# llm-d-incubation/workload-variant-autoscaler

Measured on AMD Instinct MI355X. Metric: solver_wall_clock_ms, lower is better.
Workload: dtype fp64; 1 GPU; model=3 models x 2 service classes (config #3), variants=64, accelerator_types=3, global_batch=64, seq_len=0, parallelism=fleet-shard dp1, analyzer_device=cuda

## Files before the change

### wva_amd/csrc/queue_solver.cpp

```cpp

#include <torch/extension.h>

#ifdef WVA_WITH_HIP
#include <c10/hip/HIPStream.h>
#endif

#include <climits>
#include <cmath>
#include <vector>


#include "queue_host.h"

#ifdef WVA_WITH_HIP
extern "C" int wva_launch_solve(const double *prob, double *out, int n_problems,
                                int max_k, void *stream);
#endif

static torch::Tensor solve_allocations(torch::Tensor problems, int64_t max_k_hint = -1) {
  TORCH_CHECK(problems.dim() == 2 && problems.size(1) == wva::PROBLEM_FIELDS,
              "problems must be [B, ", (int)wva::PROBLEM_FIELDS, "]");
  TORCH_CHECK(problems.scalar_type() == torch::kFloat64, "problems must be float64");
  problems = problems.contiguous();
  const int64_t B = problems.size(0);
  auto out = torch::zeros({B, (int64_t)wva::RESULT_FIELDS}, problems.options());
  if (B == 0) return out;

  if (problems.is_cuda()) {
#ifdef WVA_WITH_HIP
    int max_k;
    if (max_k_hint > 0) {
      max_k = max_k_hint > INT_MAX ? INT_MAX : (int)max_k_hint;
    } else {
      auto n = problems.select(1, wva::P_MAX_BATCH);
      auto in_range = n.ge(1.0).logical_and(n.lt((double)wva::kMaxBatchLimit + 1.0));
      const double max_batch =
          torch::where(in_range, n, torch::ones_like(n)).max().item<double>();
      max_k = (int)max_batch * (1 + wva::kMaxQueueToBatchRatio);
    }
    auto stream = c10::hip::getCurrentHIPStream();
    const int status = wva_launch_solve(problems.data_ptr<double>(),
                                        out.data_ptr<double>(), (int)B, max_k,
                                        (void *)stream.stream());
    TORCH_CHECK(status != -1,
                "max_batch too large for the LDS-resident GPU path (limit ~700, "
                "chain length ", max_k, "); use the CPU path for these problems");
    TORCH_CHECK(status == 0, "wva sizing kernel launch failed: ",
                hipGetErrorString((hipError_t)status));
    return out;
#else
    TORCH_CHECK(false, "wva native extension built without HIP support");
#endif
  }

  const double *pr = problems.data_ptr<double>();
  double *res = out.data_ptr<double>();
  int max_k = 1;
  for (int64_t i = 0; i < B; ++i) {
    int k = wva::row_chain_length(pr + i * wva::PROBLEM_FIELDS);
    if (k > max_k) max_k = k;
  }
  at::parallel_for(0, B, 1, [&](int64_t begin, int64_t end) {
    std::vector<double> cum((size_t)max_k);
    for (int64_t i = begin; i < end; ++i) {
      wva::solve_one(pr + i * wva::PROBLEM_FIELDS, res + i * wva::RESULT_FIELDS,
                     cum.data());
    }
  });
  return out;
}

PYBIND11_MODULE(TORCH_EXTENSION_NAME, m) {
  m.doc() = "wva_amd native batched queue solver (CPU + gfx950 HIP)";
  m.def("solve_allocations", &solve_allocations,
        "Batched state-dependent M/M/1/K allocation sizing",
        pybind11::arg("problems"), pybind11::arg("max_k_hint") = -1);
  m.attr("PROBLEM_FIELDS") = (int)wva::PROBLEM_FIELDS;
  m.attr("RESULT_FIELDS") = (int)wva::RESULT_FIELDS;
#ifdef WVA_WITH_HIP
  m.attr("HAS_HIP") = true;
#else
  m.attr("HAS_HIP") = false;
#endif
}
```

### wva_amd/ops/batched.py

```python

from __future__ import annotations

import math
from typing import Dict, List, Optional, Tuple

import numpy as np

from ..analyzer import (
    AnalyzerError,
    Configuration,
    DecodeParms,
    PrefillParms,
    QueueAnalyzer,
    RequestSize,
    ServiceParms,
    TargetPerf,
)
from ..config import MAX_QUEUE_TO_BATCH_RATIO
from ..core import Allocation, System
from ..core.allocation import _zero_load_allocation, energy_value_term

P_ALPHA, P_BETA, P_GAMMA, P_DELTA = 0, 1, 2, 3
P_IN_TOKENS, P_OUT_TOKENS, P_MAX_BATCH = 4, 5, 6
P_TARGET_TTFT, P_TARGET_ITL, P_TARGET_TPS = 7, 8, 9
P_TOTAL_RATE, P_MIN_REPLICAS = 10, 11
PROBLEM_FIELDS = 12

R_FEASIBLE, R_REPLICAS, R_RATE_STAR, R_ITL, R_TTFT, R_RHO = range(6)
RESULT_FIELDS = 6

GPU_MAX_BATCH_LIMIT = 700

_MAX_BATCH_LIMIT = (2**31 - 1) // (1 + MAX_QUEUE_TO_BATCH_RATIO)


def valid_rows(problems: np.ndarray) -> np.ndarray:
    p = problems
    with np.errstate(invalid="ignore"):
        ok = np.isfinite(p).all(axis=1)
        ok &= (p[:, P_ALPHA : P_DELTA + 1] >= 0).all(axis=1)
        ok &= (p[:, P_MAX_BATCH] >= 1) & (p[:, P_MAX_BATCH] < _MAX_BATCH_LIMIT + 1)
        ok &= (p[:, P_OUT_TOKENS] >= 1) & (p[:, P_OUT_TOKENS] < 2.0**31)
        ok &= p[:, P_IN_TOKENS] >= 0
        ok &= (p[:, P_TARGET_TTFT : P_TARGET_TPS + 1] >= 0).all(axis=1)
    return ok

_graph_cache: dict = {}
_graph_lock = None
_graph_disabled = False
_mg1_warned = False


def _graph_solve(native, problems_t, max_k):
    global _graph_lock, _graph_disabled
    import os
    import threading

    if _graph_disabled or os.environ.get("WVA_GPU_GRAPH", "0") != "1":
        return None
    import torch

    if _graph_lock is None:
        _graph_lock = threading.Lock()
    key = (problems_t.shape[0], max_k)
    with _graph_lock:
        entry = _graph_cache.get(key)
        try:
            if entry is None:
                if len(_graph_cache) >= 16:
                    _graph_cache.pop(next(iter(_graph_cache)))
                static_in = problems_t.clone()
                side = torch.cuda.Stream()
                side.wait_stream(torch.cuda.current_stream())
                with torch.cuda.stream(side):
                    native.solve_allocations(static_in, max_k)
                torch.cuda.current_stream().wait_stream(side)
                graph = torch.cuda.CUDAGraph()
                with torch.cuda.graph(graph):
                    static_out = native.solve_allocations(static_in, max_k)
                _graph_cache[key] = (graph, static_in, static_out)
                graph.replay()
                return static_out.cpu().numpy()
            graph, static_in, static_out = entry
            static_in.copy_(problems_t)
            graph.replay()
            return static_out.cpu().numpy()
        except Exception as e:
            _graph_disabled = True
            import logging

            logging.getLogger("wva").warning(
                "hipGraph dispatch unavailable; using plain launches: %s", e
            )
            return None


def _solve_problems_python(problems: np.ndarray, scv=1.0) -> np.ndarray:
    scv_arr = np.broadcast_to(np.asarray(scv, dtype=np.float64), (problems.shape[0],))
    out = np.zeros((problems.shape[0], RESULT_FIELDS), dtype=np.float64)
    valid = valid_rows(problems)
    for i, row in enumerate(problems):
        if not valid[i]:
            continue
        N = int(row[P_MAX_BATCH])
        config = Configuration(
            max_batch_size=N,
            max_queue_size=N * MAX_QUEUE_TO_BATCH_RATIO,
            service_parms=ServiceParms(
                prefill=PrefillParms(gamma=row[P_GAMMA], delta=row[P_DELTA]),
                decode=DecodeParms(alpha=row[P_ALPHA], beta=row[P_BETA]),
            ),
        )
        try:
            qa = QueueAnalyzer(
                config,
                RequestSize(
                    avg_input_tokens=int(row[P_IN_TOKENS]),
                    avg_output_tokens=int(row[P_OUT_TOKENS]),
                ),
                scv=float(scv_arr[i]),
            )
            _, metrics, _ = qa.size(
                TargetPerf(
                    target_ttft=row[P_TARGET_TTFT],
                    target_itl=row[P_TARGET_ITL],
                    target_tps=row[P_TARGET_TPS],
                )
            )
            rate_star = metrics.throughput
            total_rate = row[P_TOTAL_RATE]
            n_rep = max(math.ceil(total_rate / rate_star), int(row[P_MIN_REPLICAS]))
            if n_rep <= 0:
                continue
            final = qa.analyze(total_rate / n_rep)
        except AnalyzerError:
            continue
        out[i, R_FEASIBLE] = 1.0
        out[i, R_REPLICAS] = n_rep
        out[i, R_RATE_STAR] = rate_star
        out[i, R_ITL] = final.avg_token_time
        out[i, R_TTFT] = final.avg_wait_time + final.avg_prefill_time
        out[i, R_RHO] = final.rho
    return out


def solve_problems(problems: np.ndarray, device: Optional[str] = None) -> np.ndarray:
    from . import get_native, native_available

    problems = np.ascontiguousarray(problems, dtype=np.float64)
    if problems.ndim != 2 or problems.shape[1] != PROBLEM_FIELDS:
        raise ValueError(f"problems must be [B, {PROBLEM_FIELDS}]")
    if problems.shape[0] == 0:
        return np.zeros((0, RESULT_FIELDS), dtype=np.float64)

    from ..analyzer.mg1 import configured_scv

    scv = configured_scv()
    if scv != 1.0:
        global _mg1_warned
        if not _mg1_warned:
            _mg1_warned = True
            import logging

            logging.getLogger("wva_amd.ops").info(
                "WVA_ANALYZER=mg1 (cs^2=%.3g): sizing via the Python "
                "M/G/1-corrected analyzer instead of the native kernel", scv,
            )
        return _solve_problems_python(problems, scv=scv)

    want_gpu = device is not None and str(device).startswith("cuda")
    if want_gpu:
        native = get_native()
        import torch

        batch_limits = problems[:, P_MAX_BATCH]
        max_batch = batch_limits.max()
        if not max_batch <= GPU_MAX_BATCH_LIMIT:
            batch_limits = np.where(valid_rows(problems), batch_limits, 1.0)
            max_batch = batch_limits.max()
        if max_batch > GPU_MAX_BATCH_LIMIT:
            big = batch_limits > GPU_MAX_BATCH_LIMIT
            out = np.empty((problems.shape[0], RESULT_FIELDS), dtype=np.float64)
            out[~big] = solve_problems(problems[~big], device=device)
            out[big] = solve_problems(problems[big], device="cpu")
            return out
        max_k = max(int(max_batch), 1) * (1 + MAX_QUEUE_TO_BATCH_RATIO)
        t = torch.from_numpy(problems).to(device)
        res = _graph_solve(native, t, max_k)
        if res is not None:
            return res
        return native.solve_allocations(t, max_k).cpu().numpy()

    from . import get_native_cpu, native_cpu_available

    if native_cpu_available():
        return get_native_cpu().solve_allocations(problems)
    if native_available():
        import torch

        native = get_native()
        return native.solve_allocations(torch.from_numpy(problems)).numpy()
    from . import warn_if_pure_python_fallback

    warn_if_pure_python_fallback()
    return _solve_problems_python(problems)


class BatchedAllocationSolver:

    def __init__(self, device: Optional[str] = None) -> None:
        self.device = device

    def calculate(self, system: System) -> None:
        for g in system.accelerators.values():
            g.calculate()

        pair_cache: Dict[Tuple[str, str], Optional[Tuple[float, float, float, float, int, int, float]]] = {}

        def pair_info(model, acc):
            key = (model.name, acc.name)
            hit = pair_cache.get(key, False)
            if hit is not False:
                return hit
            perf = model.get_perf_data(acc.name)
            if perf is None:
                pair_cache[key] = None
                return None
            info = (
                perf.decode_parms.alpha,
                perf.decode_parms.beta,
                perf.prefill_parms.gamma,
                perf.prefill_parms.delta,
                perf.max_batch_size,
                perf.at_tokens,
                acc.cost * model.get_num_instances(acc.name),
            )
            pair_cache[key] = info
            return info

        from ..core.allocation import sizing_headroom

        headroom_factor = 1.0 + sizing_headroom()
        rows: List[Tuple[float, ...]] = []
        keys: List[Tuple[str, str, int]] = []
        zero_load: Dict[str, Dict[str, Allocation]] = {}
        costs: List[float] = []
        scv_rows: List[float] = []
        rows_append, keys_append, costs_append = rows.append, keys.append, costs.append
        scv_append = scv_rows.append

        for server in system.servers.values():
            server.all_allocations = {}
            load = server.load
            if (
                load is None
                or load.arrival_rate < 0
                or load.avg_in_tokens < 0
                or load.avg_out_tokens < 0
            ):
                continue
            model = system.model(server.model_name)
            if model is None:
                continue
            svc = system.service_class(server.service_class_name)
            if svc is None:
                continue
            target = svc.model_target(server.model_name)
            if target is None:
                continue
            target_ttft, target_itl, target_tps = target.ttft, target.itl, target.tps
            arrival, in_tok, out_tok = load.arrival_rate, load.avg_in_tokens, load.avg_out_tokens
            server_name = server.name
            server_max_batch = server.max_batch_size
            min_replicas = float(server.min_num_replicas)
            candidates = server.get_candidate_accelerators(system.accelerators)
            for acc in candidates.values():
                info = pair_info(model, acc)
                if info is None:
                    continue
                if arrival == 0 or out_tok == 0:
                    perf = model.get_perf_data(acc.name)
                    alloc = _zero_load_allocation(server, model, acc, perf)
                    zero_load.setdefault(server_name, {})[acc.name] = alloc
                    continue
                alpha, beta, gamma, delta, perf_max_batch, at_tokens, cost_per_rep = info
                K = int(out_tok)
                N = server_max_batch if server_max_batch > 0 else max(perf_max_batch * at_tokens // K, 1)
                total_rate = (
                    arrival / 60.0 if target_tps == 0 else target_tps / float(K)
                ) * headroom_factor
                rows_append(
                    (alpha, beta, gamma, delta, float(int(in_tok)), float(K), float(N),
                     target_ttft, target_itl, target_tps, total_rate, min_replicas)
                )
                keys_append((server_name, acc.name, N))
                costs_append(cost_per_rep)
                scv_append(getattr(server, "service_scv", -1.0))

        if rows:
            arr = np.array(rows, dtype=np.float64)
            from ..analyzer.mg1 import configured_scv

            global_scv = configured_scv()
            scv_arr = np.array(
                [s if s >= 0 else global_scv for s in scv_rows], dtype=np.float64
            )
            if (scv_arr != 1.0).any():
                results = _solve_problems_python(arr, scv=scv_arr)
            else:
                results = solve_problems(arr, self.device)
        else:
            results = np.zeros((0, RESULT_FIELDS))

        opt_spec = system.optimizer_spec
        energy_enabled = (
            opt_spec is not None
            and opt_spec.objective == "cost+energy"
            and opt_spec.energy_cost_per_kwh > 0
        )
        servers = system.servers
        results_list = results.tolist()
        for (server_name, acc_name, N), res, cost_per_replica in zip(keys, results_list, costs):
            if res[R_FEASIBLE] != 1.0:
                continue
            server = servers[server_name]
            num_replicas = int(res[R_REPLICAS])
            alloc = Allocation(
                accelerator=acc_name,
                num_replicas=num_replicas,
                batch_size=N,
                cost=cost_per_replica * num_replicas,
                itl=res[R_ITL],
                ttft=res[R_TTFT],
                rho=res[R_RHO],
                max_arrv_rate_per_replica=res[R_RATE_STAR] / 1000.0,
            )
            cur = server.cur_allocation
            alloc.value = cur.transition_penalty(alloc) if cur is not None else alloc.cost
            if energy_enabled:
                alloc.value += energy_value_term(system, server, alloc)
            server.all_allocations[acc_name] = alloc

        for server_name, accs in zero_load.items():
            server = servers[server_name]
            for acc_name, alloc in accs.items():
                if server.cur_allocation is not None:
                    alloc.set_value(server.cur_allocation.transition_penalty(alloc))
                if energy_enabled:
                    alloc.set_value(alloc.value + energy_value_term(system, server, alloc))
                server.all_allocations[acc_name] = alloc
```

Before: 931.4 us.

## Add pinned-buffer async GPU dispatch and chunk host row building over kernel

Adds a native submit/collect path that keeps a pool of pinned host and device buffers on a private non-blocking stream, so upload, the sizing kernel and download are queued without torch tensor allocation or a device sync per call. The batched solver splits servers into chunks (two by default for small fleets) so Python row building and result application for one chunk overlap with the GPU solve of the other. The CUDA output tensor also switches from zeros to empty. The cost is more complexity, per-slot lifetime state, and an extra kernel launch per chunk, which can outweigh the overlap when the fleet is small.

```diff
diff --git a/wva_amd/csrc/queue_solver.cpp b/wva_amd/csrc/queue_solver.cpp
--- a/wva_amd/csrc/queue_solver.cpp
+++ b/wva_amd/csrc/queue_solver.cpp
@@ -15,6 +15,8 @@
 #ifdef WVA_WITH_HIP
 extern "C" int wva_launch_solve(const double *prob, double *out, int n_problems,
                                 int max_k, void *stream);
+
+#include "sizing_dispatch.h"
 #endif
 
 static torch::Tensor solve_allocations(torch::Tensor problems, int64_t max_k_hint = -1) {
@@ -23,7 +25,9 @@
   TORCH_CHECK(problems.scalar_type() == torch::kFloat64, "problems must be float64");
   problems = problems.contiguous();
   const int64_t B = problems.size(0);
-  auto out = torch::zeros({B, (int64_t)wva::RESULT_FIELDS}, problems.options());
+  auto out = problems.is_cuda()
+                 ? torch::empty({B, (int64_t)wva::RESULT_FIELDS}, problems.options())
+                 : torch::zeros({B, (int64_t)wva::RESULT_FIELDS}, problems.options());
   if (B == 0) return out;
 
   if (problems.is_cuda()) {
@@ -78,6 +82,16 @@
   m.attr("PROBLEM_FIELDS") = (int)wva::PROBLEM_FIELDS;
   m.attr("RESULT_FIELDS") = (int)wva::RESULT_FIELDS;
 #ifdef WVA_WITH_HIP
+  m.def("submit", &wva::dispatch::submit,
+        "Enqueue upload, sizing kernel and download for a float64 [B, 12] "
+        "numpy array on the private dispatch stream; returns a ticket "
+        "without waiting",
+        pybind11::arg("problems"), pybind11::arg("max_k"));
+  m.def("collect", &wva::dispatch::collect,
+        "Wait (GIL released) for a ticket and return its float64 [B, 6] results",
+        pybind11::arg("ticket"));
+  m.def("dispatch_pool_stats", &wva::dispatch::pool_stats,
+        "(slots, slots in flight) of the dispatch pool");
   m.attr("HAS_HIP") = true;
 #else
   m.attr("HAS_HIP") = false;
diff --git a/wva_amd/csrc/sizing_dispatch.h b/wva_amd/csrc/sizing_dispatch.h
--- /dev/null
+++ b/wva_amd/csrc/sizing_dispatch.h
@@ -0,0 +1,228 @@
+
+#pragma once
+
+#include <hip/hip_runtime.h>
+#include <pybind11/numpy.h>
+#include <pybind11/pybind11.h>
+
+#include <climits>
+#include <cstdint>
+#include <cstring>
+#include <mutex>
+#include <stdexcept>
+#include <string>
+#include <unordered_set>
+#include <vector>
+
+#include "queue_core.h"
+
+extern "C" int wva_launch_solve(const double *prob, double *out, int n_problems,
+                                int max_k, void *stream);
+
+namespace wva {
+namespace dispatch {
+
+namespace py = pybind11;
+
+inline void hip_check(hipError_t err, const char *what) {
+  if (err != hipSuccess) {
+    throw std::runtime_error(std::string("wva sizing dispatch: ") + what +
+                             " failed: " + hipGetErrorString(err));
+  }
+}
+
+struct DeviceGuard {
+  int prev = -1;
+  bool switched = false;
+  explicit DeviceGuard(int device) {
+    hip_check(hipGetDevice(&prev), "hipGetDevice");
+    if (prev != device) {
+      hip_check(hipSetDevice(device), "hipSetDevice");
+      switched = true;
+    }
+  }
+  ~DeviceGuard() {
+    if (switched) (void)hipSetDevice(prev);
+  }
+};
+
+enum class SlotState { kFree, kInFlight, kCollecting };
+
+struct Slot {
+  double *h_in = nullptr;
+  double *h_out = nullptr;
+  double *d_in = nullptr;
+  double *d_out = nullptr;
+  int64_t cap_rows = 0;
+  hipEvent_t done = nullptr;
+  SlotState state = SlotState::kFree;
+  int64_t ticket = 0;
+  int64_t rows = 0;
+};
+
+struct Pool {
+  std::mutex mu;
+  int device = -1;
+  hipStream_t stream = nullptr;
+  std::vector<Slot *> slots;
+  std::unordered_set<int64_t> empty_tickets;
+  int64_t next_ticket = 1;
+};
+
+inline Pool &pool() {
+  static Pool *p = new Pool();
+  return *p;
+}
+
+inline void grow_slot(Slot &s, int64_t rows) {
+  if (rows <= s.cap_rows) return;
+  if (s.h_in) (void)hipHostFree(s.h_in);
+  if (s.h_out) (void)hipHostFree(s.h_out);
+  if (s.d_in) (void)hipFree(s.d_in);
+  if (s.d_out) (void)hipFree(s.d_out);
+  s.h_in = s.h_out = s.d_in = s.d_out = nullptr;
+  s.cap_rows = 0;
+  const int64_t cap = (rows + 255) / 256 * 256;
+  const size_t in_bytes = (size_t)cap * PROBLEM_FIELDS * sizeof(double);
+  const size_t out_bytes = (size_t)cap * RESULT_FIELDS * sizeof(double);
+  hip_check(hipHostMalloc((void **)&s.h_in, in_bytes, hipHostMallocDefault),
+            "hipHostMalloc");
+  hip_check(hipHostMalloc((void **)&s.h_out, out_bytes, hipHostMallocDefault),
+            "hipHostMalloc");
+  hip_check(hipMalloc((void **)&s.d_in, in_bytes), "hipMalloc");
+  hip_check(hipMalloc((void **)&s.d_out, out_bytes), "hipMalloc");
+  s.cap_rows = cap;
+}
+
+inline int64_t submit(py::array problems, int64_t max_k) {
+  if (!py::isinstance<py::array_t<double>>(problems)) {
+    throw py::type_error("problems must be a float64 array");
+  }
+  if (problems.ndim() != 2 || problems.shape(1) != PROBLEM_FIELDS) {
+    throw py::value_error("problems must be [B, " +
+                          std::to_string((int)PROBLEM_FIELDS) + "]");
+  }
+  if (!(problems.flags() & py::array::c_style)) {
+    throw py::value_error("problems must be C-contiguous");
+  }
+  const int64_t B = problems.shape(0);
+  if (B > INT_MAX) throw py::value_error("too many problems for one launch");
+
+  Pool &P = pool();
+  std::lock_guard<std::mutex> lock(P.mu);
+  if (B == 0) {
+    const int64_t ticket = P.next_ticket++;
+    P.empty_tickets.insert(ticket);
+    return ticket;
+  }
+  if (P.device < 0) hip_check(hipGetDevice(&P.device), "hipGetDevice");
+  DeviceGuard guard(P.device);
+  if (P.stream == nullptr) {
+    hip_check(hipStreamCreateWithFlags(&P.stream, hipStreamNonBlocking),
+              "hipStreamCreateWithFlags");
+  }
+
+  Slot *slot = nullptr;
+  for (Slot *s : P.slots) {
+    if (s->state == SlotState::kFree) {
+      slot = s;
+      break;
+    }
+  }
+  if (slot == nullptr) {
+    Slot *s = new Slot();
+    hipError_t err = hipEventCreateWithFlags(&s->done, hipEventDisableTiming);
+    if (err != hipSuccess) {
+      delete s;
+      hip_check(err, "hipEventCreateWithFlags");
+    }
+    P.slots.push_back(s);
+    slot = s;
+  }
+  grow_slot(*slot, B);
+
+  const size_t in_bytes = (size_t)B * PROBLEM_FIELDS * sizeof(double);
+  const size_t out_bytes = (size_t)B * RESULT_FIELDS * sizeof(double);
+  std::memcpy(slot->h_in, problems.data(), in_bytes);
+  hip_check(hipMemcpyAsync(slot->d_in, slot->h_in, in_bytes,
+                           hipMemcpyHostToDevice, P.stream),
+            "hipMemcpyAsync (upload)");
+  const int k = max_k > INT_MAX ? INT_MAX : (max_k < 0 ? 0 : (int)max_k);
+  const int status =
+      wva_launch_solve(slot->d_in, slot->d_out, (int)B, k, (void *)P.stream);
+  if (status != 0) {
+    (void)hipStreamSynchronize(P.stream);
+    if (status == -1) {
+      throw std::runtime_error(
+          "no kernel geometry holds a chain of length " + std::to_string(max_k) +
+          " in LDS (max_batch limit ~700); use the CPU path for these problems");
+    }
+    hip_check((hipError_t)status, "sizing kernel launch");
+  }
+  hipError_t err = hipMemcpyAsync(slot->h_out, slot->d_out, out_bytes,
+                                  hipMemcpyDeviceToHost, P.stream);
+  if (err == hipSuccess) err = hipEventRecord(slot->done, P.stream);
+  if (err != hipSuccess) {
+    (void)hipStreamSynchronize(P.stream);
+    hip_check(err, "hipMemcpyAsync (download) / hipEventRecord");
+  }
+  slot->state = SlotState::kInFlight;
+  slot->ticket = P.next_ticket++;
+  slot->rows = B;
+  return slot->ticket;
+}
+
+inline std::vector<py::ssize_t> result_shape(int64_t rows) {
+  return {(py::ssize_t)rows, (py::ssize_t)RESULT_FIELDS};
+}
+
+inline py::array_t<double> collect(int64_t ticket) {
+  Pool &P = pool();
+  Slot *slot = nullptr;
+  {
+    std::lock_guard<std::mutex> lock(P.mu);
+    if (P.empty_tickets.erase(ticket)) {
+      return py::array_t<double>(result_shape(0));
+    }
+    for (Slot *s : P.slots) {
+      if (s->ticket == ticket && s->state != SlotState::kFree) {
+        slot = s;
+        break;
+      }
+    }
+    if (slot == nullptr || slot->state == SlotState::kCollecting) {
+      const bool issued = ticket >= 1 && ticket < P.next_ticket;
+      throw py::value_error(
+          (issued ? "sizing ticket already collected: " : "unknown sizing ticket: ") +
+          std::to_string(ticket));
+    }
+    slot->state = SlotState::kCollecting;
+  }
+  const int64_t rows = slot->rows;
+  py::array_t<double> out(result_shape(rows));
+  double *dst = out.mutable_data();
+  hipError_t err;
+  {
+    py::gil_scoped_release nogil;
+    err = hipEventSynchronize(slot->done);
+    if (err == hipSuccess) {
+      std::memcpy(dst, slot->h_out, (size_t)rows * RESULT_FIELDS * sizeof(double));
+    }
+    std::lock_guard<std::mutex> lock(P.mu);
+    slot->state = SlotState::kFree;
+    slot->ticket = 0;
+  }
+  hip_check(err, "hipEventSynchronize");
+  return out;
+}
+
+inline py::tuple pool_stats() {
+  Pool &P = pool();
+  std::lock_guard<std::mutex> lock(P.mu);
+  int64_t busy = 0;
+  for (Slot *s : P.slots) busy += s->state != SlotState::kFree;
+  return py::make_tuple((int64_t)P.slots.size(), busy);
+}
+
+}
+}
diff --git a/wva_amd/ops/batched.py b/wva_amd/ops/batched.py
--- a/wva_amd/ops/batched.py
+++ b/wva_amd/ops/batched.py
@@ -1,7 +1,9 @@
 
 from __future__ import annotations
 
+import contextlib
 import math
+import os
 from typing import Dict, List, Optional, Tuple
 
 import numpy as np
@@ -51,9 +53,23 @@
 _mg1_warned = False
 
 
+def _graph_requested() -> bool:
+    return not _graph_disabled and os.environ.get("WVA_GPU_GRAPH", "0") == "1"
+
+
+_NO_DEVICE_SWITCH = contextlib.nullcontext()
+
+
+def _on_device(device):
+    if str(device) == "cuda":
+        return _NO_DEVICE_SWITCH
+    import torch
+
+    return torch.cuda.device(torch.device(device))
+
+
 def _graph_solve(native, problems_t, max_k):
     global _graph_lock, _graph_disabled
-    import os
     import threading
 
     if _graph_disabled or os.environ.get("WVA_GPU_GRAPH", "0") != "1":
@@ -185,11 +201,13 @@
             out[big] = solve_problems(problems[big], device="cpu")
             return out
         max_k = max(int(max_batch), 1) * (1 + MAX_QUEUE_TO_BATCH_RATIO)
-        t = torch.from_numpy(problems).to(device)
-        res = _graph_solve(native, t, max_k)
-        if res is not None:
-            return res
-        return native.solve_allocations(t, max_k).cpu().numpy()
+        if _graph_requested():
+            t = torch.from_numpy(problems).to(device)
+            res = _graph_solve(native, t, max_k)
+            if res is not None:
+                return res
+        with _on_device(device):
+            return native.collect(native.submit(problems, max_k))
 
     from . import get_native_cpu, native_cpu_available
 
@@ -206,14 +224,87 @@
     return _solve_problems_python(problems)
 
 
+class SyncDispatch:
+
+    def __init__(self, device: Optional[str], global_scv: Optional[float] = None) -> None:
+        self.device = device
+        self.global_scv = global_scv
+
+    def submit(self, problems: np.ndarray, scv_rows=None):
+        if self.global_scv is not None:
+            scv_arr = np.array(
+                [s if s >= 0 else self.global_scv for s in scv_rows], dtype=np.float64
+            )
+            if (scv_arr != 1.0).any():
+                return _solve_problems_python(problems, scv=scv_arr)
+        return solve_problems(problems, self.device)
+
+    def collect(self, ticket) -> np.ndarray:
+        return ticket
+
+
+class NativeGpuDispatch:
+
+    def __init__(self, native, device: str) -> None:
+        self.native = native
+        self.device = device
+
+    def submit(self, problems: np.ndarray, scv_rows=None):
+        max_batch = problems[:, P_MAX_BATCH].max()
+        if not max_batch <= GPU_MAX_BATCH_LIMIT:
+            return None, solve_problems(problems, self.device)
+        max_k = max(int(max_batch), 1) * (1 + MAX_QUEUE_TO_BATCH_RATIO)
+        with _on_device(self.device):
+            return self.native.submit(problems, max_k), None
+
+    def collect(self, ticket) -> np.ndarray:
+        native_ticket, solved = ticket
+        if native_ticket is None:
+            return solved
+        return self.native.collect(native_ticket)
+
+
+DEFAULT_GPU_CHUNKS = 2
+
+_GPU_CHUNKING_ROW_BOUND = 512
+
+
 class BatchedAllocationSolver:
 
-    def __init__(self, device: Optional[str] = None) -> None:
+    def __init__(self, device: Optional[str] = None, chunks: Optional[int] = None) -> None:
+        if chunks is not None and chunks < 1:
+            raise ValueError("chunks must be at least 1")
         self.device = device
+        self.chunks = chunks
+
+    def _plan(self, system: System, servers):
+        from ..analyzer.mg1 import configured_scv
+
+        global_scv = configured_scv()
+        if global_scv != 1.0 or any(
+            s >= 0 and s != 1.0 for s in [getattr(v, "service_scv", -1.0) for v in servers]
+        ):
+            return SyncDispatch(self.device, global_scv), 1, True
+        want_gpu = self.device is not None and str(self.device).startswith("cuda")
+        if want_gpu and not _graph_requested():
+            from . import get_native
+
+            native = get_native()
+            if native is None or not native.HAS_HIP:
+                raise RuntimeError("the native HIP extension is required for device "
+                                   f"{self.device!r} and is not built")
+            chunks = self.chunks if self.chunks is not None else DEFAULT_GPU_CHUNKS
+            if len(servers) * len(system.accelerators) >= _GPU_CHUNKING_ROW_BOUND:
+                chunks = 1
+            return NativeGpuDispatch(native, self.device), chunks, False
+        return SyncDispatch(self.device), self.chunks or 1, False
 
     def calculate(self, system: System) -> None:
         for g in system.accelerators.values():
             g.calculate()
+
+        all_servers = list(system.servers.values())
+        dispatch, n_chunks, track_scv = self._plan(system, all_servers)
 
         pair_cache: Dict[Tuple[str, str], Optional[Tuple[float, float, float, float, int, int, float]]] = {}
 
@@ -241,77 +332,7 @@
         from ..core.allocation import sizing_headroom
 
         headroom_factor = 1.0 + sizing_headroom()
-        rows: List[Tuple[float, ...]] = []
-        keys: List[Tuple[str, str, int]] = []
-        zero_load: Dict[str, Dict[str, Allocation]] = {}
-        costs: List[float] = []
-        scv_rows: List[float] = []
-        rows_append, keys_append, costs_append = rows.append, keys.append, costs.append
-        scv_append = scv_rows.append
-
-        for server in system.servers.values():
-            server.all_allocations = {}
-            load = server.load
-            if (
-                load is None
-                or load.arrival_rate < 0
-                or load.avg_in_tokens < 0
-                or load.avg_out_tokens < 0
-            ):
-                continue
-            model = system.model(server.model_name)
-            if model is None:
-                continue
-            svc = system.service_class(server.service_class_name)
-            if svc is None:
-                continue
-            target = svc.model_target(server.model_name)
-            if target is None:
-                continue
-            target_ttft, target_itl, target_tps = target.ttft, target.itl, target.tps
-            arrival, in_tok, out_tok = load.arrival_rate, load.avg_in_tokens, load.avg_out_tokens
-            server_name = server.name
-            server_max_batch = server.max_batch_size
-            min_replicas = float(server.min_num_replicas)
-            candidates = server.get_candidate_accelerators(system.accelerators)
-            for acc in candidates.values():
-                info = pair_info(model, acc)
-                if info is None:
-                    continue
-                if arrival == 0 or out_tok == 0:
-                    perf = model.get_perf_data(acc.name)
-                    alloc = _zero_load_allocation(server, model, acc, perf)
-                    zero_load.setdefault(server_name, {})[acc.name] = alloc
-                    continue
-                alpha, beta, gamma, delta, perf_max_batch, at_tokens, cost_per_rep = info
-                K = int(out_tok)
-                N = server_max_batch if server_max_batch > 0 else max(perf_max_batch * at_tokens // K, 1)
-                total_rate = (
-                    arrival / 60.0 if target_tps == 0 else target_tps / float(K)
-                ) * headroom_factor
-                rows_append(
-                    (alpha, beta, gamma, delta, float(int(in_tok)), float(K), float(N),
-                     target_ttft, target_itl, target_tps, total_rate, min_replicas)
-                )
-                keys_append((server_name, acc.name, N))
-                costs_append(cost_per_rep)
-                scv_append(getattr(server, "service_scv", -1.0))
-
-        if rows:
-            arr = np.array(rows, dtype=np.float64)
-            from ..analyzer.mg1 import configured_scv
-
-            global_scv = configured_scv()
-            scv_arr = np.array(
-                [s if s >= 0 else global_scv for s in scv_rows], dtype=np.float64
-            )
-            if (scv_arr != 1.0).any():
-                results = _solve_problems_python(arr, scv=scv_arr)
-            else:
-                results = solve_problems(arr, self.device)
-        else:
-            results = np.zeros((0, RESULT_FIELDS))
-
+        accelerators = system.accelerators
         opt_spec = system.optimizer_spec
         energy_enabled = (
             opt_spec is not None
@@ -319,33 +340,124 @@
             and opt_spec.energy_cost_per_kwh > 0
         )
         servers = system.servers
-        results_list = results.tolist()
-        for (server_name, acc_name, N), res, cost_per_replica in zip(keys, results_list, costs):
-            if res[R_FEASIBLE] != 1.0:
-                continue
-            server = servers[server_name]
-            num_replicas = int(res[R_REPLICAS])
-            alloc = Allocation(
-                accelerator=acc_name,
-                num_replicas=num_replicas,
-                batch_size=N,
-                cost=cost_per_replica * num_replicas,
-                itl=res[R_ITL],
-                ttft=res[R_TTFT],
-                rho=res[R_RHO],
-                max_arrv_rate_per_replica=res[R_RATE_STAR] / 1000.0,
-            )
-            cur = server.cur_allocation
-            alloc.value = cur.transition_penalty(alloc) if cur is not None else alloc.cost
-            if energy_enabled:
-                alloc.value += energy_value_term(system, server, alloc)
-            server.all_allocations[acc_name] = alloc
-
-        for server_name, accs in zero_load.items():
-            server = servers[server_name]
-            for acc_name, alloc in accs.items():
-                if server.cur_allocation is not None:
-                    alloc.set_value(server.cur_allocation.transition_penalty(alloc))
+
+        def build_rows(chunk_servers):
+            rows: List[Tuple[float, ...]] = []
+            keys: List[Tuple[str, str, int]] = []
+            zero_load: Dict[str, Dict[str, Allocation]] = {}
+            costs: List[float] = []
+            scv_rows: List[float] = []
+            rows_append, keys_append, costs_append = rows.append, keys.append, costs.append
+            scv_append = scv_rows.append
+
+            for server in chunk_servers:
+                server.all_allocations = {}
+                load = server.load
+                if (
+                    load is None
+                    or load.arrival_rate < 0
+                    or load.avg_in_tokens < 0
+                    or load.avg_out_tokens < 0
+                ):
+                    continue
+                model = system.model(server.model_name)
+                if model is None:
+                    continue
+                svc = system.service_class(server.service_class_name)
+                if svc is None:
+                    continue
+                target = svc.model_target(server.model_name)
+                if target is None:
+                    continue
+                target_ttft, target_itl, target_tps = target.ttft, target.itl, target.tps
+                arrival, in_tok, out_tok = load.arrival_rate, load.avg_in_tokens, load.avg_out_tokens
+                server_name = server.name
+                server_max_batch = server.max_batch_size
+                min_replicas = float(server.min_num_replicas)
+                candidates = server.get_candidate_accelerators(accelerators)
+                for acc in candidates.values():
+                    info = pair_info(model, acc)
+                    if info is None:
+                        continue
+                    if arrival == 0 or out_tok == 0:
+                        perf = model.get_perf_data(acc.name)
+                        alloc = _zero_load_allocation(server, model, acc, perf)
+                        zero_load.setdefault(server_name, {})[acc.name] = alloc
+                        continue
+                    alpha, beta, gamma, delta, perf_max_batch, at_tokens, cost_per_rep = info
+                    K = int(out_tok)
+                    N = server_max_batch if server_max_batch > 0 else max(perf_max_batch * at_tokens // K, 1)
+                    total_rate = (
+                        arrival / 60.0 if target_tps == 0 else target_tps / float(K)
+                    ) * headroom_factor
+                    rows_append(
+                        (alpha, beta, gamma, delta, float(int(in_tok)), float(K), float(N),
+                         target_ttft, target_itl, target_tps, total_rate, min_replicas)
+                    )
+                    keys_append((server_name, acc.name, N))
+                    costs_append(cost_per_rep)
+                    if track_scv:
+                        scv_append(getattr(server, "service_scv", -1.0))
+
+            ticket = None
+            if rows:
+                ticket = dispatch.submit(np.array(rows, dtype=np.float64), scv_rows)
+            return ticket, keys, costs, zero_load
+
+        def apply_results(ticket, keys, costs, zero_load):
+            if ticket is not None:
+                results_list = dispatch.collect(ticket).tolist()
+            else:
+                results_list = []
+            for (server_name, acc_name, N), res, cost_per_replica in zip(keys, results_list, costs):
+                if res[R_FEASIBLE] != 1.0:
+                    continue
+                server = servers[server_name]
+                num_replicas = int(res[R_REPLICAS])
+                alloc = Allocation(
+                    accelerator=acc_name,
+                    num_replicas=num_replicas,
+                    batch_size=N,
+                    cost=cost_per_replica * num_replicas,
+                    itl=res[R_ITL],
+                    ttft=res[R_TTFT],
+                    rho=res[R_RHO],
+                    max_arrv_rate_per_replica=res[R_RATE_STAR] / 1000.0,
+                )
+                cur = server.cur_allocation
+                alloc.value = cur.transition_penalty(alloc) if cur is not None else alloc.cost
                 if energy_enabled:
-                    alloc.set_value(alloc.value + energy_value_term(system, server, alloc))
+                    alloc.value += energy_value_term(system, server, alloc)
                 server.all_allocations[acc_name] = alloc
+
+            for server_name, accs in zero_load.items():
+                server = servers[server_name]
+                for acc_name, alloc in accs.items():
+                    if server.cur_allocation is not None:
+                        alloc.set_value(server.cur_allocation.transition_penalty(alloc))
+                    if energy_enabled:
+                        alloc.set_value(alloc.value + energy_value_term(system, server, alloc))
+                    server.all_allocations[acc_name] = alloc
+
+        n = len(all_servers)
+        bounds = [n * i // n_chunks for i in range(n_chunks + 1)]
+        pending = None
+        try:
+            for lo, hi in zip(bounds, bounds[1:]):
+                if lo == hi:
+                    continue
+                submitted = build_rows(all_servers[lo:hi])
+                if pending is not None:
+                    previous, pending = pending, submitted
+                    apply_results(*previous)
+                else:
+                    pending = submitted
+            if pending is not None:
+                last, pending = pending, None
+                apply_results(*last)
+        finally:
+            if pending is not None and pending[0] is not None:
+                try:
+                    dispatch.collect(pending[0])
+                except Exception:
+                    pass
```

After: 839.2 us (median of 6 runs). 9.9% less time.
